# llm-d/llm-d-workload-variant-autoscaler

Measured on AMD Instinct MI355X. Metric: desired-replica accuracy + SLO-attainment %, Llama-3-8B synthetic QPS ramp, higher is better.
Workload: dtype bf16; 1 GPU; model=meta-llama/Llama-3.1-8B, global_batch=256, seq_len=150, parallelism=dp1, device=AMD Radeon Graphics

## Files before the change

### wva_amd/ops/csrc/attention.hip

```cpp
#include "common.h"

#include <type_traits>

#define HEAD_DIM 128
#define MAX_G 8
#define TILE 64
#define NUM_WAVES 4
#define ROW_DW 66
#define S_ROW 65

template <bool KV_FP8>
using kv_elem_t = std::conditional_t<KV_FP8, fp8_t, bf16>;

__device__ __forceinline__ long ws_row_offset(int b, int kvh, int g, int split,
                                              int num_kv_heads, int G,
                                              int num_splits) {
  return ((((long)b * num_kv_heads + kvh) * G + g) * num_splits + split) *
         (2 + HEAD_DIM);
}

__device__ __forceinline__ long pack8_fp8(const float* v, float inv_scale) {
  unsigned int lo = 0, hi = 0;
  lo = __builtin_amdgcn_cvt_pk_fp8_f32(v[0] * inv_scale, v[1] * inv_scale,
                                       lo, false);
// ... 35 lines not shown
#pragma unroll
      for (int i = 0; i < 8; ++i) {
        qf.bf[kk][i] = src[i];
        const bf16 bv = *reinterpret_cast<const bf16*>(&src[i]);
        qv[kk][i] = bf2f(bv);
      }
    }
  } else {
#pragma unroll
    for (int kk = 0; kk < 4; ++kk)
#pragma unroll
      for (int i = 0; i < 8; ++i) qf.bf[kk][i] = 0;
  }
  if constexpr (KV_FP8) {
    float amax = 0.0f;
#pragma unroll
    for (int kk = 0; kk < 4; ++kk)
#pragma unroll
      for (int i = 0; i < 8; ++i) amax = fmaxf(amax, fabsf(qv[kk][i]));
    amax = wave_reduce_max(amax);
    if (lane == 0) qmax_lds[wave] = amax;
    __syncthreads();
    float m0 = qmax_lds[0];
#pragma unroll
    for (int w2 = 1; w2 < NUM_WAVES; ++w2) m0 = fmaxf(m0, qmax_lds[w2]);
    qf.scale = fmaxf(m0 / 448.0f, 1e-12f);
    const float inv = 1.0f / qf.scale;
#pragma unroll
    for (int kk = 0; kk < 4; ++kk) qf.fp8[kk] = pack8_fp8(qv[kk], inv);
    __syncthreads();
  }
  return qf;
}

struct SoftmaxStep {
  float p;
  float corr;
};

__device__ __forceinline__ SoftmaxStep online_softmax_step(
    const float* __restrict__ s_row, int tn, int lane, float& m, float& s) {
  const bool live = lane < tn;
  const float score = live ? s_row[lane] : -INFINITY;
  const float tile_max = wave_reduce_max(score);
  const float m_new = fmaxf(m, tile_max);
  const float p = live ? __expf(score - m_new) : 0.0f;
  const float tile_sum = wave_reduce_sum(p);
  const float corr = (m == -INFINITY) ? 0.0f : __expf(m - m_new);
  s = s * corr + tile_sum;
  m = m_new;
  return {p, corr};
}

template <bool KV_FP8>
__global__ __launch_bounds__(256, 2) void gqa_decode_attn_v4_kernel(
    bf16* __restrict__ out,
    float* __restrict__ workspace,
    const bf16* __restrict__ q,
    const void* __restrict__ k_cache,
    const void* __restrict__ v_cache,
    const int* __restrict__ context_lens,
    const int num_q_heads,
    const int num_kv_heads,
    const int max_seq,
    const float scale) {
  const int b = blockIdx.x;
  const int kvh = blockIdx.y;
  const int split = blockIdx.z;
  const int num_splits = gridDim.z;
  const int G = num_q_heads / num_kv_heads;
  const int ctx = context_lens[b];

  const int lane = threadIdx.x & (WAVE_SIZE - 1);
  const int wave = threadIdx.x / WAVE_SIZE;
  const int frag_col = lane % 16;
  const int frag_k0 = 8 * (lane / 16);

  __shared__ float s_smem[MAX_G][S_ROW];
  __shared__ unsigned int v_smem[TILE * ROW_DW];
  __shared__ float p_smem[MAX_G][TILE];
  float* qmax_lds = nullptr;
  if constexpr (KV_FP8) {
    __shared__ float qmax_smem[NUM_WAVES];
    qmax_lds = qmax_smem;
  }

  const QFrags qf = load_q_frags<KV_FP8>(q, b, kvh, G, num_q_heads, lane,
                                         wave, frag_col, frag_k0, qmax_lds);

  const int heads_mine = (G > wave) ? (G - wave + NUM_WAVES - 1) / NUM_WAVES : 0;
  float m[2], s[2], acc[2][2];
#pragma unroll
  for (int j = 0; j < 2; ++j) {
    m[j] = -INFINITY;
    s[j] = 0.0f;
    acc[j][0] = acc[j][1] = 0.0f;
  }

  const long slab_off = ((long)b * num_kv_heads + kvh) * max_seq * HEAD_DIM;
  const auto* k_slab =
      reinterpret_cast<const kv_elem_t<KV_FP8>*>(k_cache) + slab_off;
  const auto* v_slab =
      reinterpret_cast<const kv_elem_t<KV_FP8>*>(v_cache) + slab_off;

  for (int t0 = split * TILE; t0 < ctx; t0 += num_splits * TILE) {
    const int tn = min(TILE, ctx - t0);

    if constexpr (KV_FP8) {
      const int tile_g8 = tn * (HEAD_DIM / 8);
      const fp8_t* v_src = v_slab + (long)t0 * HEAD_DIM;
      for (int idx = wave * WAVE_SIZE + lane; idx < tile_g8;
           idx += NUM_WAVES * WAVE_SIZE) {
        const int row = idx >> 4;
        const int d8 = (idx & 15) * 8;
        const unsigned short* src =
            reinterpret_cast<const unsigned short*>(
                v_src + (long)row * HEAD_DIM + d8);
        unsigned int* dst = &v_smem[row * ROW_DW + d8 / 2];
#pragma unroll
        for (int j = 0; j < 4; ++j) {
          const float2_vt f = unpk2_fp8(src[j]);
          const bf16x2 packed{f2bf(f[0]), f2bf(f[1])};
          dst[j] = *reinterpret_cast<const unsigned int*>(&packed);
        }
      }
    } else {
      typedef __attribute__((ext_vector_type(2))) unsigned int uint2_t;
      const int tile_u2 = tn * (HEAD_DIM / 4);
      const unsigned int* v_src =
          reinterpret_cast<const unsigned int*>(v_slab + (long)t0 * HEAD_DIM);
      for (int idx = wave * WAVE_SIZE + lane; idx < tile_u2;
           idx += NUM_WAVES * WAVE_SIZE) {
        const int row = idx >> 5;
        const int d2 = (idx & 31) * 2;
        const uint2_t val = *reinterpret_cast<const uint2_t*>(&v_src[idx * 2]);
        *reinterpret_cast<uint2_t*>(&v_smem[row * ROW_DW + d2]) = val;
      }
    }

    {
      const int prow = 16 * wave + (lane % 16);
      const int pos = t0 + prow;
      const int pos_c = pos < max_seq ? pos : max_seq - 1;
      const int k0 = frag_k0;
      f32x4_frag sf = {0.f, 0.f, 0.f, 0.f};
      if constexpr (KV_FP8) {
        const long* ksrc = reinterpret_cast<const long*>(
            k_slab + (long)pos_c * HEAD_DIM);
        const int l0 = k0 / 8;
#pragma unroll
        for (int kk = 0; kk < 4; ++kk) {
          const long a8 = ksrc[kk * 4 + l0];
          sf = __builtin_amdgcn_mfma_f32_16x16x32_fp8_fp8(
              a8, qf.fp8[kk], sf, 0, 0, 0);
        }
      } else {
#pragma unroll
        for (int kk = 0; kk < 4; ++kk) {
          bf16x8_frag a_frag;
          const short* src = reinterpret_cast<const short*>(
              k_slab + (long)pos_c * HEAD_DIM) + 32 * kk + k0;
#pragma unroll
          for (int i = 0; i < 8; ++i) a_frag[i] = src[i];
          sf = __builtin_amdgcn_mfma_f32_16x16x32_bf16(a_frag, qf.bf[kk],
                                                       sf, 0, 0, 0);
        }
      }
      const float s_eff = KV_FP8 ? scale * qf.scale : scale;
      const int g = lane & 15;
      if (g < G) {
#pragma unroll
        for (int i = 0; i < 4; ++i) {
          const int t = 16 * wave + (lane >> 4) * 4 + i;
          s_smem[g][t] = (t < tn) ? sf[i] * s_eff : -INFINITY;
        }
      }
    }
    __syncthreads();

    for (int j = 0; j < heads_mine; ++j) {
      const int g = wave + j * NUM_WAVES;
      const SoftmaxStep st = online_softmax_step(s_smem[g], tn, lane, m[j], s[j]);
      acc[j][0] *= st.corr;
      acc[j][1] *= st.corr;
      p_smem[g][lane] = st.p;
    }

    for (int j = 0; j < heads_mine; ++j) {
      const int g = wave + j * NUM_WAVES;
      const float* pg = p_smem[g];
      float a0 = acc[j][0], a1 = acc[j][1];
      for (int t = 0; t < tn; ++t) {
        const unsigned int vw = v_smem[t * ROW_DW + lane];
        const bf16x2 vv = *reinterpret_cast<const bf16x2*>(&vw);
        const float p = pg[t];
        a0 = fmaf(p, bf2f(vv.x), a0);
        a1 = fmaf(p, bf2f(vv.y), a1);
      }
      acc[j][0] = a0;
      acc[j][1] = a1;
    }
    __syncthreads();
  }

  if (num_splits == 1) {
    for (int j = 0; j < heads_mine; ++j) {
      const int g = wave + j * NUM_WAVES;
      const float inv = s[j] > 0.0f ? 1.0f / s[j] : 0.0f;
      bf16x2* orow = reinterpret_cast<bf16x2*>(
          out + ((long)b * num_q_heads + kvh * G + g) * HEAD_DIM);
      orow[lane] = bf16x2{f2bf(acc[j][0] * inv), f2bf(acc[j][1] * inv)};
    }
  } else {
    for (int j = 0; j < heads_mine; ++j) {
      const int g = wave + j * NUM_WAVES;
      float* wsp = workspace +
          ws_row_offset(b, kvh, g, split, num_kv_heads, G, num_splits);
      if (lane == 0) {
        wsp[0] = m[j];
        wsp[1] = s[j];
      }
      wsp[2 + 2 * lane] = acc[j][0];
      wsp[2 + 2 * lane + 1] = acc[j][1];
    }
  }
}

template <bool KV_FP8>
__global__ __launch_bounds__(256, 2) void gqa_decode_attn_v5_kernel(
    bf16* __restrict__ out,
    float* __restrict__ workspace,
    const bf16* __restrict__ q,
    const void* __restrict__ k_cache,
    const void* __restrict__ v_cache,
    const int* __restrict__ context_lens,
    const int num_q_heads,
    const int num_kv_heads,
    const int max_seq,
    const float scale) {
  const int b = blockIdx.x;
  const int kvh = blockIdx.y;
  const int split = blockIdx.z;
  const int num_splits = gridDim.z;
  const int G = num_q_heads / num_kv_heads;
  const int ctx = context_lens[b];

  const int lane = threadIdx.x & (WAVE_SIZE - 1);
  const int wave = threadIdx.x / WAVE_SIZE;
  const int frag_col = lane % 16;
  const int frag_k0 = 8 * (lane / 16);

  __shared__ float s_smem[MAX_G][S_ROW];
  __shared__ unsigned int v_smem[TILE * ROW_DW];
  __shared__ float p_smem[MAX_G][TILE];
  __shared__ float corr_smem[MAX_G];
  __shared__ float sum_smem[MAX_G];
  __shared__ float m_smem[MAX_G];
  float* qmax_lds = nullptr;
  if constexpr (KV_FP8) {
    __shared__ float qmax_smem[NUM_WAVES];
    qmax_lds = qmax_smem;
  }

  const QFrags qf = load_q_frags<KV_FP8>(q, b, kvh, G, num_q_heads, lane,
                                         wave, frag_col, frag_k0, qmax_lds);

  const int heads_mine = (G > wave) ? (G - wave + NUM_WAVES - 1) / NUM_WAVES : 0;
  float m[2], s[2];
#pragma unroll
  for (int j = 0; j < 2; ++j) {
    m[j] = -INFINITY;
    s[j] = 0.0f;
  }
  f32x4_frag acc_pv[2] = {f32x4_frag{0.f, 0.f, 0.f, 0.f},
                          f32x4_frag{0.f, 0.f, 0.f, 0.f}};

  const long slab_off = ((long)b * num_kv_heads + kvh) * max_seq * HEAD_DIM;
  const auto* k_slab =
      reinterpret_cast<const kv_elem_t<KV_FP8>*>(k_cache) + slab_off;
  const auto* v_slab =
      reinterpret_cast<const kv_elem_t<KV_FP8>*>(v_cache) + slab_off;

  for (int t0 = split * TILE; t0 < ctx; t0 += num_splits * TILE) {
    const int tn = min(TILE, ctx - t0);

    if constexpr (KV_FP8) {
      const int tile_g8 = tn * (HEAD_DIM / 8);
      const fp8_t* v_src = v_slab + (long)t0 * HEAD_DIM;
      for (int idx = wave * WAVE_SIZE + lane; idx < tile_g8;
           idx += NUM_WAVES * WAVE_SIZE) {
        const int row = idx >> 4;
        const int d8 = (idx & 15) * 8;
        const unsigned short* src =
            reinterpret_cast<const unsigned short*>(
                v_src + (long)row * HEAD_DIM + d8);
        unsigned int* dst = &v_smem[row * ROW_DW + d8 / 2];
#pragma unroll
        for (int j = 0; j < 4; ++j) {
          const float2_vt f = unpk2_fp8(src[j]);
          const bf16x2 packed{f2bf(f[0]), f2bf(f[1])};
          dst[j] = *reinterpret_cast<const unsigned int*>(&packed);
        }
      }
    } else {
      typedef __attribute__((ext_vector_type(2))) unsigned int uint2_t;
      const int tile_u2 = tn * (HEAD_DIM / 4);
      const unsigned int* v_src =
          reinterpret_cast<const unsigned int*>(v_slab + (long)t0 * HEAD_DIM);
      for (int idx = wave * WAVE_SIZE + lane; idx < tile_u2;
           idx += NUM_WAVES * WAVE_SIZE) {
        const int row = idx >> 5;
        const int d2 = (idx & 31) * 2;
        const uint2_t val = *reinterpret_cast<const uint2_t*>(&v_src[idx * 2]);
        *reinterpret_cast<uint2_t*>(&v_smem[row * ROW_DW + d2]) = val;
      }
    }

    {
      const int prow = 16 * wave + (lane % 16);
      const int pos = t0 + prow;
      const int pos_c = pos < max_seq ? pos : max_seq - 1;
      const int k0 = frag_k0;
      f32x4_frag sf = {0.f, 0.f, 0.f, 0.f};
      if constexpr (KV_FP8) {
        const long* ksrc = reinterpret_cast<const long*>(
            k_slab + (long)pos_c * HEAD_DIM);
        const int l0 = k0 / 8;
#pragma unroll
        for (int kk = 0; kk < 4; ++kk) {
          const long a8 = ksrc[kk * 4 + l0];
          sf = __builtin_amdgcn_mfma_f32_16x16x32_fp8_fp8(
              a8, qf.fp8[kk], sf, 0, 0, 0);
        }
      } else {
#pragma unroll
        for (int kk = 0; kk < 4; ++kk) {
          bf16x8_frag a_frag;
          const short* src = reinterpret_cast<const short*>(
              k_slab + (long)pos_c * HEAD_DIM) + 32 * kk + k0;
#pragma unroll
          for (int i = 0; i < 8; ++i) a_frag[i] = src[i];
          sf = __builtin_amdgcn_mfma_f32_16x16x32_bf16(a_frag, qf.bf[kk],
                                                       sf, 0, 0, 0);
        }
      }
      const float s_eff = KV_FP8 ? scale * qf.scale : scale;
      const int g = lane & 15;
      if (g < G) {
#pragma unroll
        for (int i = 0; i < 4; ++i) {
          const int t = 16 * wave + (lane >> 4) * 4 + i;
          s_smem[g][t] = (t < tn) ? sf[i] * s_eff : -INFINITY;
        }
      }
    }
    __syncthreads();

    for (int j = 0; j < heads_mine; ++j) {
      const int g = wave + j * NUM_WAVES;
      const SoftmaxStep st = online_softmax_step(s_smem[g], tn, lane, m[j], s[j]);
      p_smem[g][lane] = st.p;
      if (lane == 0) corr_smem[g] = st.corr;
    }
    __syncthreads();

    {
      bf16x8_frag p_frag[2];
#pragma unroll
      for (int kk = 0; kk < 2; ++kk) {
        const int g = lane % 16;
        const int pos0 = 32 * kk + 8 * (lane / 16);
        if (g < G) {
#pragma unroll
          for (int i = 0; i < 8; ++i)
            p_frag[kk][i] = f2bf_bits(p_smem[g][pos0 + i]);
        } else {
#pragma unroll
          for (int i = 0; i < 8; ++i) p_frag[kk][i] = 0;
        }
      }
      const unsigned short* v_u16 =
          reinterpret_cast<const unsigned short*>(v_smem);
#pragma unroll
      for (int nsub = 0; nsub < 2; ++nsub) {
        const int dim = 16 * (wave + 4 * nsub) + (lane % 16);
        f32x4_frag d = acc_pv[nsub];
#pragma unroll
        for (int i = 0; i < 4; ++i) {
          const int h = (lane >> 4) * 4 + i;
          d[i] *= (h < G) ? corr_smem[h] : 0.0f;
        }
#pragma unroll
        for (int kk = 0; kk < 2; ++kk) {
          bf16x8_frag v_frag;
          const int pos0 = 32 * kk + 8 * (lane / 16);
#pragma unroll
          for (int i = 0; i < 8; ++i) {
            const int t = pos0 + i;
            v_frag[i] = (t < tn)
                ? (short)v_u16[(t * ROW_DW + (dim >> 1)) * 2 + (dim & 1)]
                : (short)0;
          }
          d = __builtin_amdgcn_mfma_f32_16x16x32_bf16(p_frag[kk], v_frag, d,
                                                      0, 0, 0);
        }
        acc_pv[nsub] = d;
      }
    }
    __syncthreads();
  }

  for (int j = 0; j < heads_mine; ++j) {
    const int g = wave + j * NUM_WAVES;
    if (lane == 0) {
      sum_smem[g] = s[j];
      m_smem[g] = m[j];
    }
  }
  __syncthreads();

  if (num_splits == 1) {
#pragma unroll
    for (int nsub = 0; nsub < 2; ++nsub) {
      const int dim = 16 * (wave + 4 * nsub) + (lane & 15);
#pragma unroll
      for (int i = 0; i < 4; ++i) {
        const int h = (lane >> 4) * 4 + i;
        if (h >= G) continue;
        const float sv = sum_smem[h];
        const float inv = sv > 0.0f ? 1.0f / sv : 0.0f;
        out[((long)b * num_q_heads + kvh * G + h) * HEAD_DIM + dim] =
            f2bf(acc_pv[nsub][i] * inv);
      }
    }
  } else {
#pragma unroll
    for (int nsub = 0; nsub < 2; ++nsub) {
      const int dim = 16 * (wave + 4 * nsub) + (lane & 15);
#pragma unroll
      for (int i = 0; i < 4; ++i) {
        const int h = (lane >> 4) * 4 + i;
        if (h >= G) continue;
        float* wsp = workspace +
            ws_row_offset(b, kvh, h, split, num_kv_heads, G, num_splits);
        if (wave == 0 && nsub == 0 && (lane & 15) == 0) {
          wsp[0] = m_smem[h];
          wsp[1] = sum_smem[h];
        }
        wsp[2 + dim] = acc_pv[nsub][i];
      }
    }
  }
}

#define MERGE_WAVES 8
// ... 7 lines not shown
  const int h = blockIdx.y;
  const int G = num_q_heads / num_kv_heads;
  const int kvh = h / G;
  const int g = h % G;
  const int lane = threadIdx.x & 63;
  const int wave = threadIdx.x >> 6;

  __shared__ float sm_m[MERGE_WAVES];
  __shared__ float sm_s[MERGE_WAVES];
  __shared__ float sm_o[MERGE_WAVES][HEAD_DIM];

  const float* base = workspace +
      ws_row_offset(b, kvh, g, 0, num_kv_heads, G, num_splits);
  float M = -INFINITY;
  for (int sp = wave; sp < num_splits; sp += MERGE_WAVES) {
    M = fmaxf(M, base[sp * (2 + HEAD_DIM)]);
  }
  float S = 0.0f, o0 = 0.0f, o1 = 0.0f;
  for (int sp = wave; sp < num_splits; sp += MERGE_WAVES) {
    const float* wsp = base + sp * (2 + HEAD_DIM);
    const float mw = wsp[0];
    if (mw == -INFINITY) continue;
    const float f = __expf(mw - M);
    S += wsp[1] * f;
    o0 = fmaf(wsp[2 + 2 * lane], f, o0);
    o1 = fmaf(wsp[2 + 2 * lane + 1], f, o1);
  }
  if (lane == 0) {
    sm_m[wave] = M;
    sm_s[wave] = S;
  }
  sm_o[wave][2 * lane] = o0;
  sm_o[wave][2 * lane + 1] = o1;
  __syncthreads();

  if (wave != 0) return;
  float Mg = -INFINITY;
  for (int w = 0; w < MERGE_WAVES; ++w) Mg = fmaxf(Mg, sm_m[w]);
  float Sg = 0.0f;
  float g0 = 0.0f, g1 = 0.0f;
  for (int w = 0; w < MERGE_WAVES; ++w) {
    if (sm_m[w] == -INFINITY) continue;
    const float f = __expf(sm_m[w] - Mg);
    Sg += sm_s[w] * f;
    g0 = fmaf(sm_o[w][2 * lane], f, g0);
    g1 = fmaf(sm_o[w][2 * lane + 1], f, g1);
  }
  const float inv = Sg > 0.0f ? 1.0f / Sg : 0.0f;
  bf16x2* orow = reinterpret_cast<bf16x2*>(
      out + ((long)b * num_q_heads + h) * HEAD_DIM);
  orow[lane] = bf16x2{f2bf(g0 * inv), f2bf(g1 * inv)};
}

extern "C" int gqa_decode_attn_num_splits(int batch, int num_kv_heads,
                                          int max_ctx_hint) {
  const int base = batch * num_kv_heads;
  if (base >= 1792) return 1;
  int splits = 1792 / base;
  static int min_tiles = [] {
    const char* e = getenv("WVA_ATTN_MIN_TILES");
    int v = e ? atoi(e) : 8;
    return v > 0 ? v : 8;
  }();
  int cap = 16;
  if (max_ctx_hint > 0) {
    const int by_work = max_ctx_hint / (min_tiles * TILE);
    if (by_work > cap) cap = by_work;
  }
  if (splits > cap) splits = cap;
  const int max_useful = max_ctx_hint > 0 ? (max_ctx_hint + 2 * TILE - 1) / (2 * TILE) : splits;
  if (splits > max_useful && max_useful >= 1) splits = max_useful;
  return splits < 1 ? 1 : splits;
}

extern "C" void launch_gqa_decode_attn(
    void* out, void* workspace, const void* q, const void* k_cache,
    const void* v_cache, const int* context_lens, int batch, int num_q_heads,
    int num_kv_heads, int max_seq, int num_splits, float scale, int variant,
    int kv_fp8, hipStream_t stream) {
  const auto kernel =
      variant == 5 ? (kv_fp8 ? gqa_decode_attn_v5_kernel<true>
                             : gqa_decode_attn_v5_kernel<false>)
                   : (kv_fp8 ? gqa_decode_attn_v4_kernel<true>
                             : gqa_decode_attn_v4_kernel<false>);
  hipLaunchKernelGGL(kernel, dim3(batch, num_kv_heads, num_splits), dim3(256),
                     0, stream, (bf16*)out, (float*)workspace, (const bf16*)q,
                     k_cache, v_cache, context_lens, num_q_heads, num_kv_heads,
                     max_seq, scale);
  if (num_splits > 1) {
    hipLaunchKernelGGL(gqa_decode_attn_merge_kernel,
                       dim3(batch, num_q_heads), dim3(64 * MERGE_WAVES), 0,
                       stream, (bf16*)out, (const float*)workspace,
                       num_q_heads, num_kv_heads, num_splits);
  }
}
```

### wva_amd/ops/csrc/ops.cpp

```cpp

#include <torch/extension.h>
#include <hip/hip_runtime.h>
#include <c10/hip/HIPStream.h>

#include <string>

extern "C" void launch_rmsnorm(void* out, void* residual_out,
                               const void* input, const void* residual,
                               const void* weight, float eps, int rows,
                               int hidden, hipStream_t stream);
extern "C" void launch_rope(void* q, void* k, const int* positions, int tokens,
                            int num_q_heads, int num_k_heads, int head_dim,
                            float theta, hipStream_t stream);
extern "C" void launch_silu_mul(void* out, const void* gate, const void* up,
                                long n, hipStream_t stream);
extern "C" void launch_silu_mul_fused(void* out, const void* gate_up,
                                      long rows, long inter,
                                      hipStream_t stream);
extern "C" void launch_rope_append_kv_fp8(const void* qkv, void* q_out,
                                          void* k_cache, void* v_cache,
                                          const int* positions, int batch,
                                          int num_q_heads, int num_kv_heads,
                                          int head_dim, int max_seq,
                                          float theta, hipStream_t stream);
extern "C" void launch_rope_append_kv(const void* qkv, void* q_out,
                                      void* k_cache, void* v_cache,
                                      const int* positions, int batch,
                                      int num_q_heads, int num_kv_heads,
                                      int head_dim, int max_seq, float theta,
                                      hipStream_t stream);
extern "C" int gqa_decode_attn_num_splits(int batch, int num_kv_heads,
                                          int max_ctx_hint);
extern "C" int skinny_gemm_num_splits(int N, int K, int nt);
extern "C" void launch_prefill_attn_ex(void* out, const void* q,
                                       const void* k_cache,
                                       const void* v_cache, int batch,
                                       int seq, int num_q_heads,
                                       int num_kv_heads, int max_seq,
                                       float scale, int kv_fp8,
                                       hipStream_t stream);
extern "C" int skinny_gemm_tile_n(int M);
extern "C" void launch_skinny_gemm(void* c, void* ws, const void* a,
                                   const void* w, int M, int N, int K,
                                   int num_splits, hipStream_t stream);
extern "C" void launch_skinny_gemm_ex(void* c, void* ws, const void* a,
                                      const void* w, const float* w_scale,
                                      int M, int N, int K, int num_splits,
                                      int w_fp8, hipStream_t stream);
extern "C" void launch_gqa_decode_attn(void* out, void* workspace,
                                       const void* q, const void* k_cache,
                                       const void* v_cache,
                                       const int* context_lens, int batch,
                                       int num_q_heads, int num_kv_heads,
                                       int max_seq, int num_splits,
                                       float scale, int variant, int kv_fp8,
                                       hipStream_t stream);

extern "C" int moe_num_m_tiles(int TK, int E);
extern "C" int moe_down_num_splits(int TK, int E, int H, int I);
extern "C" void launch_moe_route(int* topk_idx, float* topk_w,
                                 int* expert_offsets, int* sorted_slots,
                                 const float* logits, int T, int E, int K,
                                 hipStream_t stream);
extern "C" void launch_moe_gate_up_swiglu(void* act, const void* x,
                                          const void* w,
                                          const int* expert_offsets,
                                          const int* sorted_slots, int T,
                                          int E, int top_k, int H, int I,
                                          hipStream_t stream);
extern "C" void launch_moe_down_combine(void* out, float* ws,
                                        const void* act, const void* w,
                                        const float* topk_w,
                                        const int* expert_offsets,
                                        const int* sorted_slots, int T,
                                        int E, int top_k, int H, int I,
                                        int num_splits, hipStream_t stream);

namespace {

hipStream_t current_stream() {
  return c10::hip::getCurrentHIPStream().stream();
}

void check_bf16_contig(const torch::Tensor& t, const char* name) {
  TORCH_CHECK(t.is_cuda(), name, " must be on GPU");
// ... 87 lines not shown
         (int)num_q_heads, (int)num_kv_heads, head_dim, max_seq,
         (float)theta, current_stream());
  return q_out;
}

torch::Tensor silu_mul_fused(torch::Tensor gate_up) {
  check_bf16_contig(gate_up, "gate_up");
  TORCH_CHECK(gate_up.dim() == 2 && gate_up.size(1) % 4 == 0,
              "gate_up must be [rows, 2*inter], inter even");
  const long rows = gate_up.size(0);
  const long inter = gate_up.size(1) / 2;
  auto out = torch::empty({rows, inter}, gate_up.options());
  launch_silu_mul_fused(out.data_ptr(), gate_up.data_ptr(), rows, inter,
                        current_stream());
  return out;
}

enum class AttnVariant { Auto, V4, V5 };

AttnVariant parse_attn_variant(const std::string& name) {
  TORCH_CHECK(name == "auto" || name == "v4" || name == "v5",
              "variant must be \"auto\", \"v4\" or \"v5\", got \"", name, "\"");
  return name == "v4"   ? AttnVariant::V4
         : name == "v5" ? AttnVariant::V5
                        : AttnVariant::Auto;
}

torch::Tensor gqa_decode_attn(torch::Tensor q, torch::Tensor k_cache,
                              torch::Tensor v_cache,
                              torch::Tensor context_lens, double scale,
                              const std::string& variant_name) {
  AttnVariant variant = parse_attn_variant(variant_name);
  check_bf16_contig(q, "q");
  const bool kv_fp8 = check_cache_contig(k_cache, "k_cache");
  TORCH_CHECK(check_cache_contig(v_cache, "v_cache") == kv_fp8,
              "k/v cache dtype mismatch");
  TORCH_CHECK(context_lens.is_cuda() &&
                  context_lens.scalar_type() == torch::kInt32,
              "context_lens must be int32 on GPU");
  TORCH_CHECK(q.dim() == 3, "q must be [B, Hq, D]");
  TORCH_CHECK(k_cache.dim() == 4,
              "k_cache must be [B, Hk, S, D] (head-major)");
  const int batch = q.size(0);
  const int num_q_heads = q.size(1);
  const int head_dim = q.size(2);
  const int num_kv_heads = k_cache.size(1);
  const int max_seq = k_cache.size(2);
  TORCH_CHECK(head_dim == 128, "head_dim must be 128 (Llama-3 family)");
  TORCH_CHECK(num_q_heads % num_kv_heads == 0, "Hq must divide by Hk");
  const int G = num_q_heads / num_kv_heads;
  TORCH_CHECK(G <= 8, "GQA group size must be <= 8");
  TORCH_CHECK(v_cache.sizes() == k_cache.sizes(), "k/v cache mismatch");
  auto out = torch::empty_like(q);
  const int num_splits =
      gqa_decode_attn_num_splits(batch, num_kv_heads, max_seq);
  if (variant == AttnVariant::Auto) {
    variant = (G >= 8 || num_splits == 1) ? AttnVariant::V5 : AttnVariant::V4;
  }
  torch::Tensor workspace;
  void* ws_ptr = nullptr;
  if (num_splits > 1) {
    workspace = torch::empty(
        {(long)batch * num_kv_heads * G * num_splits * (2 + head_dim)},
        q.options().dtype(torch::kFloat32));
    ws_ptr = workspace.data_ptr();
  }
  launch_gqa_decode_attn(out.data_ptr(), ws_ptr, q.data_ptr(),
                         k_cache.data_ptr(), v_cache.data_ptr(),
                         context_lens.data_ptr<int>(), batch, num_q_heads,
                         num_kv_heads, max_seq, num_splits, (float)scale,
                         variant == AttnVariant::V5 ? 5 : 4, kv_fp8 ? 1 : 0,
                         current_stream());
  return out;
}

torch::Tensor skinny_linear(torch::Tensor x, torch::Tensor w) {
  check_bf16_contig(x, "x");
  check_bf16_contig(w, "w");
  TORCH_CHECK(x.dim() == 2 && w.dim() == 2, "x [M,K], w [N,K]");
  const int M = x.size(0);
  const int K = x.size(1);
  const int N = w.size(0);
  TORCH_CHECK(w.size(1) == K, "K mismatch");
  TORCH_CHECK(M <= 64, "skinny_linear requires M <= 64");
  TORCH_CHECK(K % 128 == 0, "K must be a multiple of 128");
  auto y = torch::empty({M, N}, x.options());
  const int nt = skinny_gemm_tile_n(M);
  const int sk = skinny_gemm_num_splits(N, K, nt);
  torch::Tensor ws;
  void* ws_ptr = nullptr;
  if (sk > 1) {
    ws = torch::empty({(long)sk * M * N},
                      x.options().dtype(torch::kFloat32));
    ws_ptr = ws.data_ptr();
  }
  launch_skinny_gemm(y.data_ptr(), ws_ptr, x.data_ptr(), w.data_ptr(), M, N,
                     K, sk, current_stream());
  return y;
}

torch::Tensor skinny_linear_fp8(torch::Tensor x, torch::Tensor w,
                                torch::Tensor w_scale) {
  check_bf16_contig(x, "x");
  TORCH_CHECK(w.is_cuda() && w.is_contiguous() &&
                  w.scalar_type() == at::kFloat8_e4m3fn,
              "w must be contiguous float8_e4m3fn");
  TORCH_CHECK(w_scale.is_cuda() && w_scale.scalar_type() == torch::kFloat &&
                  w_scale.numel() == w.size(0),
              "w_scale must be float32 [N]");
  TORCH_CHECK(x.dim() == 2 && w.dim() == 2, "x [M,K], w [N,K]");
// ... 212 lines not shown
```

### wva_amd/ops/csrc/rope.hip

```cpp

#include "common.h"

__device__ __forceinline__ void rotate_pair(
    const bf16* src, bf16* dst, int d, int half, int head_dim, float pos,
    float theta) {
  const float inv_freq = __powf(theta, -2.0f * (float)d / (float)head_dim);
  const float angle = pos * inv_freq;
  float c, s;
  __sincosf(angle, &s, &c);
  const float x1 = bf2f(src[d]);
  const float x2 = bf2f(src[d + half]);
  dst[d] = f2bf(x1 * c - x2 * s);
  dst[d + half] = f2bf(x2 * c + x1 * s);
}

__global__ void rope_kernel(
    bf16* __restrict__ q,
    bf16* __restrict__ k,
    const int* __restrict__ positions,
    const int num_q_heads,
    const int num_k_heads,
    const int head_dim,
    const float theta) {
  const int token = blockIdx.x;
  const float pos = (float)positions[token];
  const int half = head_dim / 2;
  const int total = (num_q_heads + num_k_heads) * half;

  for (int idx = threadIdx.x; idx < total; idx += blockDim.x) {
    const int head = idx / half;
    const int d = idx % half;
    const bool is_q = head < num_q_heads;
    bf16* base = is_q
        ? q + (long)token * num_q_heads * head_dim + (long)head * head_dim
        : k + (long)token * num_k_heads * head_dim +
              (long)(head - num_q_heads) * head_dim;
    rotate_pair(base, base, d, half, head_dim, pos, theta);
  }
}

__global__ void rope_append_kv_kernel(
    const bf16* __restrict__ qkv,
    bf16* __restrict__ q_out,
    bf16* __restrict__ k_cache,
    bf16* __restrict__ v_cache,
    const int* __restrict__ positions,
    const int num_q_heads,
    const int num_kv_heads,
    const int head_dim,
    const int max_seq,
    const float theta) {
  const int b = blockIdx.x;
  const int pos_i = positions[b];
  const float pos = (float)pos_i;
  const int half = head_dim / 2;
  const long qkv_row = (long)b * (num_q_heads + 2 * num_kv_heads) * head_dim;

  const int rot_total = (num_q_heads + num_kv_heads) * half;
  for (int idx = threadIdx.x; idx < rot_total; idx += blockDim.x) {
    const int head = idx / half;
    const int d = idx % half;
    if (head < num_q_heads) {
      const bf16* src = qkv + qkv_row + (long)head * head_dim;
      bf16* dst = q_out + ((long)b * num_q_heads + head) * head_dim;
      rotate_pair(src, dst, d, half, head_dim, pos, theta);
    } else {
      const int kh = head - num_q_heads;
      const bf16* src = qkv + qkv_row + ((long)num_q_heads + kh) * head_dim;
      bf16* dst = k_cache +
          (((long)b * num_kv_heads + kh) * max_seq + pos_i) * head_dim;
      rotate_pair(src, dst, d, half, head_dim, pos, theta);
    }
  }
  const int v_total = num_kv_heads * half;
  const bf16x2* vsrc = reinterpret_cast<const bf16x2*>(
      qkv + qkv_row + (long)(num_q_heads + num_kv_heads) * head_dim);
  for (int idx = threadIdx.x; idx < v_total; idx += blockDim.x) {
    const int kh = idx / half;
    const int d2 = idx % half;
    bf16x2* dst = reinterpret_cast<bf16x2*>(
        v_cache + (((long)b * num_kv_heads + kh) * max_seq + pos_i) * head_dim);
    dst[d2] = vsrc[(long)kh * half + d2];
  }
}

__global__ void rope_append_kv_fp8_kernel(
    const bf16* __restrict__ qkv,
    bf16* __restrict__ q_out,
    fp8_t* __restrict__ k_cache,
    fp8_t* __restrict__ v_cache,
    const int* __restrict__ positions,
    const int num_q_heads,
    const int num_kv_heads,
    const int head_dim,
    const int max_seq,
    const float theta) {
  const int b = blockIdx.x;
  const int pos_i = positions[b];
  const float pos = (float)pos_i;
  const int half = head_dim / 2;
  const long qkv_row = (long)b * (num_q_heads + 2 * num_kv_heads) * head_dim;

  const int rot_total = (num_q_heads + num_kv_heads) * half;
  for (int idx = threadIdx.x; idx < rot_total; idx += blockDim.x) {
    const int head = idx / half;
    const int d = idx % half;
    if (head < num_q_heads) {
      const bf16* src = qkv + qkv_row + (long)head * head_dim;
      bf16* dst = q_out + ((long)b * num_q_heads + head) * head_dim;
      rotate_pair(src, dst, d, half, head_dim, pos, theta);
    } else {
      const int kh = head - num_q_heads;
      const bf16* src = qkv + qkv_row + ((long)num_q_heads + kh) * head_dim;
      const float inv_freq =
          __powf(theta, -2.0f * (float)d / (float)head_dim);
      const float angle = pos * inv_freq;
      float c, s;
      __sincosf(angle, &s, &c);
      const float x1 = bf2f(src[d]);
      const float x2 = bf2f(src[d + half]);
      fp8_t* dst = k_cache +
          (((long)b * num_kv_heads + kh) * max_seq + pos_i) * head_dim;
      dst[d] = f2fp8(x1 * c - x2 * s);
      dst[d + half] = f2fp8(x2 * c + x1 * s);
    }
  }
  const int v_total = num_kv_heads * half;
  const bf16x2* vsrc = reinterpret_cast<const bf16x2*>(
      qkv + qkv_row + (long)(num_q_heads + num_kv_heads) * head_dim);
  for (int idx = threadIdx.x; idx < v_total; idx += blockDim.x) {
    const int kh = idx / half;
    const int d2 = idx % half;
    const bf16x2 v2 = vsrc[(long)kh * half + d2];
    unsigned short* dst = reinterpret_cast<unsigned short*>(
        v_cache + (((long)b * num_kv_heads + kh) * max_seq + pos_i) * head_dim);
    dst[d2] = pk2_fp8(bf2f(v2.x), bf2f(v2.y));
  }
}

extern "C" void launch_rope_append_kv_fp8(
    const void* qkv, void* q_out, void* k_cache, void* v_cache,
    const int* positions, int batch, int num_q_heads, int num_kv_heads,
    int head_dim, int max_seq, float theta, hipStream_t stream) {
  dim3 grid(batch);
  dim3 block(256);
  hipLaunchKernelGGL(rope_append_kv_fp8_kernel, grid, block, 0, stream,
                     (const bf16*)qkv, (bf16*)q_out, (fp8_t*)k_cache,
                     (fp8_t*)v_cache, positions, num_q_heads, num_kv_heads,
                     head_dim, max_seq, theta);
}

extern "C" void launch_rope(
    void* q, void* k, const int* positions, int tokens, int num_q_heads,
    int num_k_heads, int head_dim, float theta, hipStream_t stream) {
  dim3 grid(tokens);
  dim3 block(256);
  hipLaunchKernelGGL(rope_kernel, grid, block, 0, stream, (bf16*)q, (bf16*)k,
                     positions, num_q_heads, num_k_heads, head_dim, theta);
}

extern "C" void launch_rope_append_kv(
    const void* qkv, void* q_out, void* k_cache, void* v_cache,
    const int* positions, int batch, int num_q_heads, int num_kv_heads,
    int head_dim, int max_seq, float theta, hipStream_t stream) {
  dim3 grid(batch);
  dim3 block(256);
  hipLaunchKernelGGL(rope_append_kv_kernel, grid, block, 0, stream,
                     (const bf16*)qkv, (bf16*)q_out, (bf16*)k_cache,
                     (bf16*)v_cache, positions, num_q_heads, num_kv_heads,
                     head_dim, max_seq, theta);
}
```

Baseline: 91.98 %.

## Prefetch KV tiles into registers, use LDS transpose reads, occupancy-based splits, per-head rope

Decode attention now issues the K and V global loads for the next tile into registers right after the score barrier, so memory latency overlaps with the softmax and PV work. V5 reads V fragments with ds_read_tr16 transpose loads instead of scalar gathers. Split count now comes from a runtime occupancy query rather than a hardcoded 1792 workgroups, and the v4 kernel gets a waves-per-EU hint. The rope/append kernel is rewritten to one wave per head on a 2D grid and merged into a single template. The register prefetch raises VGPR pressure, which could lower occupancy.

```diff
diff --git a/wva_amd/ops/csrc/attention.hip b/wva_amd/ops/csrc/attention.hip
--- a/wva_amd/ops/csrc/attention.hip
+++ b/wva_amd/ops/csrc/attention.hip
@@ -111,8 +111,79 @@
   return {p, corr};
 }
 
+typedef __attribute__((ext_vector_type(2))) unsigned int uint2_t;
+
 template <bool KV_FP8>
-__global__ __launch_bounds__(256, 2) void gqa_decode_attn_v4_kernel(
+struct KVTile {
+  static constexpr int ROW_BYTES = HEAD_DIM * (int)sizeof(kv_elem_t<KV_FP8>);
+  static constexpr int V_ROWS = NUM_WAVES * WAVE_SIZE * 8 / ROW_BYTES;
+  static constexpr int V_LOADS = TILE / V_ROWS;
+  static constexpr int V_THREADS_PER_ROW = ROW_BYTES / 8;
+  using k_frag_t = std::conditional_t<KV_FP8, long, bf16x8_frag>;
+  uint2_t v[V_LOADS];
+  k_frag_t k[4];
+};
+
+template <bool KV_FP8, bool WITH_V = true, bool WITH_K = true>
+__device__ __forceinline__ void issue_tile_loads(
+    KVTile<KV_FP8>& r, const kv_elem_t<KV_FP8>* __restrict__ k_slab,
+    const kv_elem_t<KV_FP8>* __restrict__ v_slab, int t0, int tn, int max_seq,
+    int tid, int k_row, int k0) {
+  using T = KVTile<KV_FP8>;
+  const int v_r0 = tid / T::V_THREADS_PER_ROW;
+  const char* v_col = reinterpret_cast<const char*>(v_slab) +
+                      (long)t0 * T::ROW_BYTES +
+                      (tid % T::V_THREADS_PER_ROW) * 8;
+  if constexpr (WITH_V) {
+#pragma unroll
+    for (int i = 0; i < T::V_LOADS; ++i) {
+      const int row = min(v_r0 + T::V_ROWS * i, tn - 1);
+      r.v[i] = *reinterpret_cast<const uint2_t*>(v_col + row * T::ROW_BYTES);
+    }
+  }
+  const int pos = t0 + k_row;
+  const int pos_c = pos < max_seq ? pos : max_seq - 1;
+  const char* k_src = reinterpret_cast<const char*>(k_slab) +
+                      (long)pos_c * T::ROW_BYTES +
+                      k0 * (int)sizeof(kv_elem_t<KV_FP8>);
+  if constexpr (WITH_K) {
+#pragma unroll
+    for (int kk = 0; kk < 4; ++kk)
+      r.k[kk] = *reinterpret_cast<const typename T::k_frag_t*>(
+          k_src + 32 * kk * (int)sizeof(kv_elem_t<KV_FP8>));
+  }
+}
+
+template <bool KV_FP8>
+__device__ __forceinline__ void stage_v_tile(unsigned int* v_smem,
+                                             const KVTile<KV_FP8>& r, int tn,
+                                             int tid) {
+  using T = KVTile<KV_FP8>;
+  const int v_r0 = tid / T::V_THREADS_PER_ROW;
+  const int dw = (tid % T::V_THREADS_PER_ROW) * (KV_FP8 ? 4 : 2);
+  unsigned int* dst0 = &v_smem[v_r0 * ROW_DW + dw];
+#pragma unroll
+  for (int i = 0; i < T::V_LOADS; ++i) {
+    const bool live = v_r0 + T::V_ROWS * i < tn;
+    unsigned int* dst = dst0 + T::V_ROWS * i * ROW_DW;
+    if constexpr (KV_FP8) {
+#pragma unroll
+      for (int j = 0; j < 4; ++j) {
+        const unsigned int w = live ? r.v[i][j >> 1] : 0u;
+        const float2_vt f =
+            unpk2_fp8((unsigned short)((j & 1) ? (w >> 16) : (w & 0xffffu)));
+        const bf16x2 packed{f2bf(f[0]), f2bf(f[1])};
+        dst[j] = *reinterpret_cast<const unsigned int*>(&packed);
+      }
+    } else {
+      *reinterpret_cast<uint2_t*>(dst) = live ? r.v[i] : uint2_t{0u, 0u};
+    }
+  }
+}
+
+template <bool KV_FP8>
+__global__ __launch_bounds__(256) __attribute__((amdgpu_waves_per_eu(5)))
+void gqa_decode_attn_v4_kernel(
     bf16* __restrict__ out,
     float* __restrict__ workspace,
     const bf16* __restrict__ q,
@@ -162,66 +233,32 @@
   const auto* v_slab =
       reinterpret_cast<const kv_elem_t<KV_FP8>*>(v_cache) + slab_off;
 
+  const int k_row = 16 * wave + frag_col;
+  constexpr bool AHEAD_V = KV_FP8;
+  KVTile<KV_FP8> kv;
+  if (split * TILE < ctx)
+    issue_tile_loads<KV_FP8, AHEAD_V, true>(kv, k_slab, v_slab, split * TILE,
+                             min(TILE, ctx - split * TILE), max_seq,
+                             threadIdx.x, k_row, frag_k0);
+
   for (int t0 = split * TILE; t0 < ctx; t0 += num_splits * TILE) {
     const int tn = min(TILE, ctx - t0);
 
-    if constexpr (KV_FP8) {
-      const int tile_g8 = tn * (HEAD_DIM / 8);
-      const fp8_t* v_src = v_slab + (long)t0 * HEAD_DIM;
-      for (int idx = wave * WAVE_SIZE + lane; idx < tile_g8;
-           idx += NUM_WAVES * WAVE_SIZE) {
-        const int row = idx >> 4;
-        const int d8 = (idx & 15) * 8;
-        const unsigned short* src =
-            reinterpret_cast<const unsigned short*>(
-                v_src + (long)row * HEAD_DIM + d8);
-        unsigned int* dst = &v_smem[row * ROW_DW + d8 / 2];
-#pragma unroll
-        for (int j = 0; j < 4; ++j) {
-          const float2_vt f = unpk2_fp8(src[j]);
-          const bf16x2 packed{f2bf(f[0]), f2bf(f[1])};
-          dst[j] = *reinterpret_cast<const unsigned int*>(&packed);
-        }
-      }
-    } else {
-      typedef __attribute__((ext_vector_type(2))) unsigned int uint2_t;
-      const int tile_u2 = tn * (HEAD_DIM / 4);
-      const unsigned int* v_src =
-          reinterpret_cast<const unsigned int*>(v_slab + (long)t0 * HEAD_DIM);
-      for (int idx = wave * WAVE_SIZE + lane; idx < tile_u2;
-           idx += NUM_WAVES * WAVE_SIZE) {
-        const int row = idx >> 5;
-        const int d2 = (idx & 31) * 2;
-        const uint2_t val = *reinterpret_cast<const uint2_t*>(&v_src[idx * 2]);
-        *reinterpret_cast<uint2_t*>(&v_smem[row * ROW_DW + d2]) = val;
-      }
-    }
+    if constexpr (!AHEAD_V)
+      issue_tile_loads<KV_FP8, true, false>(kv, k_slab, v_slab, t0, tn,
+                                            max_seq, threadIdx.x, k_row,
+                                            frag_k0);
+    stage_v_tile<KV_FP8>(v_smem, kv, tn, threadIdx.x);
 
     {
-      const int prow = 16 * wave + (lane % 16);
-      const int pos = t0 + prow;
-      const int pos_c = pos < max_seq ? pos : max_seq - 1;
-      const int k0 = frag_k0;
       f32x4_frag sf = {0.f, 0.f, 0.f, 0.f};
-      if constexpr (KV_FP8) {
-        const long* ksrc = reinterpret_cast<const long*>(
-            k_slab + (long)pos_c * HEAD_DIM);
-        const int l0 = k0 / 8;
-#pragma unroll
-        for (int kk = 0; kk < 4; ++kk) {
-          const long a8 = ksrc[kk * 4 + l0];
+#pragma unroll
+      for (int kk = 0; kk < 4; ++kk) {
+        if constexpr (KV_FP8) {
           sf = __builtin_amdgcn_mfma_f32_16x16x32_fp8_fp8(
-              a8, qf.fp8[kk], sf, 0, 0, 0);
-        }
-      } else {
-#pragma unroll
-        for (int kk = 0; kk < 4; ++kk) {
-          bf16x8_frag a_frag;
-          const short* src = reinterpret_cast<const short*>(
-              k_slab + (long)pos_c * HEAD_DIM) + 32 * kk + k0;
-#pragma unroll
-          for (int i = 0; i < 8; ++i) a_frag[i] = src[i];
-          sf = __builtin_amdgcn_mfma_f32_16x16x32_bf16(a_frag, qf.bf[kk],
+              kv.k[kk], qf.fp8[kk], sf, 0, 0, 0);
+        } else {
+          sf = __builtin_amdgcn_mfma_f32_16x16x32_bf16(kv.k[kk], qf.bf[kk],
                                                        sf, 0, 0, 0);
         }
       }
@@ -236,6 +273,11 @@
       }
     }
     __syncthreads();
+    if (t0 + num_splits * TILE < ctx) {
+      const int t1 = t0 + num_splits * TILE;
+      issue_tile_loads<KV_FP8, AHEAD_V, true>(kv, k_slab, v_slab, t1, min(TILE, ctx - t1),
+                               max_seq, threadIdx.x, k_row, frag_k0);
+    }
 
     for (int j = 0; j < heads_mine; ++j) {
       const int g = wave + j * NUM_WAVES;
@@ -310,7 +352,7 @@
   const int frag_k0 = 8 * (lane / 16);
 
   __shared__ float s_smem[MAX_G][S_ROW];
-  __shared__ unsigned int v_smem[TILE * ROW_DW];
+  __shared__ __attribute__((aligned(16))) unsigned int v_smem[TILE * ROW_DW];
   __shared__ float p_smem[MAX_G][TILE];
   __shared__ float corr_smem[MAX_G];
   __shared__ float sum_smem[MAX_G];
@@ -340,66 +382,27 @@
   const auto* v_slab =
       reinterpret_cast<const kv_elem_t<KV_FP8>*>(v_cache) + slab_off;
 
+  const int k_row = 16 * wave + frag_col;
+  KVTile<KV_FP8> kv;
+  if (split * TILE < ctx)
+    issue_tile_loads<KV_FP8>(kv, k_slab, v_slab, split * TILE,
+                             min(TILE, ctx - split * TILE), max_seq,
+                             threadIdx.x, k_row, frag_k0);
+
   for (int t0 = split * TILE; t0 < ctx; t0 += num_splits * TILE) {
     const int tn = min(TILE, ctx - t0);
 
-    if constexpr (KV_FP8) {
-      const int tile_g8 = tn * (HEAD_DIM / 8);
-      const fp8_t* v_src = v_slab + (long)t0 * HEAD_DIM;
-      for (int idx = wave * WAVE_SIZE + lane; idx < tile_g8;
-           idx += NUM_WAVES * WAVE_SIZE) {
-        const int row = idx >> 4;
-        const int d8 = (idx & 15) * 8;
-        const unsigned short* src =
-            reinterpret_cast<const unsigned short*>(
-                v_src + (long)row * HEAD_DIM + d8);
-        unsigned int* dst = &v_smem[row * ROW_DW + d8 / 2];
-#pragma unroll
-        for (int j = 0; j < 4; ++j) {
-          const float2_vt f = unpk2_fp8(src[j]);
-          const bf16x2 packed{f2bf(f[0]), f2bf(f[1])};
-          dst[j] = *reinterpret_cast<const unsigned int*>(&packed);
-        }
-      }
-    } else {
-      typedef __attribute__((ext_vector_type(2))) unsigned int uint2_t;
-      const int tile_u2 = tn * (HEAD_DIM / 4);
-      const unsigned int* v_src =
-          reinterpret_cast<const unsigned int*>(v_slab + (long)t0 * HEAD_DIM);
-      for (int idx = wave * WAVE_SIZE + lane; idx < tile_u2;
-           idx += NUM_WAVES * WAVE_SIZE) {
-        const int row = idx >> 5;
-        const int d2 = (idx & 31) * 2;
-        const uint2_t val = *reinterpret_cast<const uint2_t*>(&v_src[idx * 2]);
-        *reinterpret_cast<uint2_t*>(&v_smem[row * ROW_DW + d2]) = val;
-      }
-    }
+    stage_v_tile<KV_FP8>(v_smem, kv, tn, threadIdx.x);
 
     {
-      const int prow = 16 * wave + (lane % 16);
-      const int pos = t0 + prow;
-      const int pos_c = pos < max_seq ? pos : max_seq - 1;
-      const int k0 = frag_k0;
       f32x4_frag sf = {0.f, 0.f, 0.f, 0.f};
-      if constexpr (KV_FP8) {
-        const long* ksrc = reinterpret_cast<const long*>(
-            k_slab + (long)pos_c * HEAD_DIM);
-        const int l0 = k0 / 8;
-#pragma unroll
-        for (int kk = 0; kk < 4; ++kk) {
-          const long a8 = ksrc[kk * 4 + l0];
+#pragma unroll
+      for (int kk = 0; kk < 4; ++kk) {
+        if constexpr (KV_FP8) {
           sf = __builtin_amdgcn_mfma_f32_16x16x32_fp8_fp8(
-              a8, qf.fp8[kk], sf, 0, 0, 0);
-        }
-      } else {
-#pragma unroll
-        for (int kk = 0; kk < 4; ++kk) {
-          bf16x8_frag a_frag;
-          const short* src = reinterpret_cast<const short*>(
-              k_slab + (long)pos_c * HEAD_DIM) + 32 * kk + k0;
-#pragma unroll
-          for (int i = 0; i < 8; ++i) a_frag[i] = src[i];
-          sf = __builtin_amdgcn_mfma_f32_16x16x32_bf16(a_frag, qf.bf[kk],
+              kv.k[kk], qf.fp8[kk], sf, 0, 0, 0);
+        } else {
+          sf = __builtin_amdgcn_mfma_f32_16x16x32_bf16(kv.k[kk], qf.bf[kk],
                                                        sf, 0, 0, 0);
         }
       }
@@ -414,6 +417,11 @@
       }
     }
     __syncthreads();
+    if (t0 + num_splits * TILE < ctx) {
+      const int t1 = t0 + num_splits * TILE;
+      issue_tile_loads<KV_FP8>(kv, k_slab, v_slab, t1, min(TILE, ctx - t1),
+                               max_seq, threadIdx.x, k_row, frag_k0);
+    }
 
     for (int j = 0; j < heads_mine; ++j) {
       const int g = wave + j * NUM_WAVES;
@@ -438,11 +446,15 @@
           for (int i = 0; i < 8; ++i) p_frag[kk][i] = 0;
         }
       }
+      typedef __attribute__((ext_vector_type(4))) short short4_t;
+      typedef __attribute__((address_space(3))) short4_t lds_short4_t;
       const unsigned short* v_u16 =
           reinterpret_cast<const unsigned short*>(v_smem);
+      const unsigned short* v_tr =
+          v_u16 + (8 * (lane / 16) + ((lane & 15) >> 2)) * (ROW_DW * 2) +
+          4 * (lane & 3);
 #pragma unroll
       for (int nsub = 0; nsub < 2; ++nsub) {
-        const int dim = 16 * (wave + 4 * nsub) + (lane % 16);
         f32x4_frag d = acc_pv[nsub];
 #pragma unroll
         for (int i = 0; i < 4; ++i) {
@@ -451,15 +463,14 @@
         }
 #pragma unroll
         for (int kk = 0; kk < 2; ++kk) {
-          bf16x8_frag v_frag;
-          const int pos0 = 32 * kk + 8 * (lane / 16);
-#pragma unroll
-          for (int i = 0; i < 8; ++i) {
-            const int t = pos0 + i;
-            v_frag[i] = (t < tn)
-                ? (short)v_u16[(t * ROW_DW + (dim >> 1)) * 2 + (dim & 1)]
-                : (short)0;
-          }
+          const unsigned short* blk =
+              v_tr + 32 * kk * (ROW_DW * 2) + 16 * (wave + 4 * nsub);
+          const short4_t lo = __builtin_amdgcn_ds_read_tr16_b64_v4i16(
+              (lds_short4_t*)blk);
+          const short4_t hi = __builtin_amdgcn_ds_read_tr16_b64_v4i16(
+              (lds_short4_t*)(blk + 4 * (ROW_DW * 2)));
+          const bf16x8_frag v_frag = {lo[0], lo[1], lo[2], lo[3],
+                                      hi[0], hi[1], hi[2], hi[3]};
           d = __builtin_amdgcn_mfma_f32_16x16x32_bf16(p_frag[kk], v_frag, d,
                                                       0, 0, 0);
         }
@@ -573,11 +584,48 @@
   orow[lane] = bf16x2{f2bf(g0 * inv), f2bf(g1 * inv)};
 }
 
+using attn_kernel_t = void (*)(bf16*, float*, const bf16*, const void*,
+                               const void*, const int*, int, int, int, float);
+
+static attn_kernel_t attn_kernel(int variant, int kv_fp8) {
+  return variant == 5 ? (kv_fp8 ? gqa_decode_attn_v5_kernel<true>
+                                : gqa_decode_attn_v5_kernel<false>)
+                      : (kv_fp8 ? gqa_decode_attn_v4_kernel<true>
+                                : gqa_decode_attn_v4_kernel<false>);
+}
+
+static int attn_resident_workgroups(int variant, int kv_fp8) {
+  struct Table {
+    int wgs[2][2];
+    Table() {
+      int dev = 0, cus = 0;
+      const bool ok =
+          hipGetDevice(&dev) == hipSuccess &&
+          hipDeviceGetAttribute(&cus, hipDeviceAttributeMultiprocessorCount,
+                                dev) == hipSuccess;
+      for (int v5 = 0; v5 < 2; ++v5)
+        for (int f8 = 0; f8 < 2; ++f8) {
+          int per_cu = 0;
+          if (!ok || hipOccupancyMaxActiveBlocksPerMultiprocessor(
+                         &per_cu, attn_kernel(v5 ? 5 : 4, f8),
+                         NUM_WAVES * WAVE_SIZE, 0) != hipSuccess)
+            per_cu = 0;
+          wgs[v5][f8] = per_cu * cus;
+        }
+    }
+  };
+  static const Table table;
+  return table.wgs[variant == 5][kv_fp8 != 0];
+}
+
 extern "C" int gqa_decode_attn_num_splits(int batch, int num_kv_heads,
-                                          int max_ctx_hint) {
+                                          int max_ctx_hint, int variant,
+                                          int kv_fp8) {
+  const int target = attn_resident_workgroups(variant, kv_fp8);
+  if (target <= 0) return 0;
   const int base = batch * num_kv_heads;
-  if (base >= 1792) return 1;
-  int splits = 1792 / base;
+  if (base >= target) return 1;
+  int splits = target / base;
   static int min_tiles = [] {
     const char* e = getenv("WVA_ATTN_MIN_TILES");
     int v = e ? atoi(e) : 8;
@@ -599,11 +647,7 @@
     const void* v_cache, const int* context_lens, int batch, int num_q_heads,
     int num_kv_heads, int max_seq, int num_splits, float scale, int variant,
     int kv_fp8, hipStream_t stream) {
-  const auto kernel =
-      variant == 5 ? (kv_fp8 ? gqa_decode_attn_v5_kernel<true>
-                             : gqa_decode_attn_v5_kernel<false>)
-                   : (kv_fp8 ? gqa_decode_attn_v4_kernel<true>
-                             : gqa_decode_attn_v4_kernel<false>);
+  const attn_kernel_t kernel = attn_kernel(variant, kv_fp8);
   hipLaunchKernelGGL(kernel, dim3(batch, num_kv_heads, num_splits), dim3(256),
                      0, stream, (bf16*)out, (float*)workspace, (const bf16*)q,
                      k_cache, v_cache, context_lens, num_q_heads, num_kv_heads,
diff --git a/wva_amd/ops/csrc/ops.cpp b/wva_amd/ops/csrc/ops.cpp
--- a/wva_amd/ops/csrc/ops.cpp
+++ b/wva_amd/ops/csrc/ops.cpp
@@ -30,7 +30,8 @@
                                       int head_dim, int max_seq, float theta,
                                       hipStream_t stream);
 extern "C" int gqa_decode_attn_num_splits(int batch, int num_kv_heads,
-                                          int max_ctx_hint);
+                                          int max_ctx_hint, int variant,
+                                          int kv_fp8);
 extern "C" int skinny_gemm_num_splits(int N, int K, int nt);
 extern "C" void launch_prefill_attn_ex(void* out, const void* q,
                                        const void* k_cache,
@@ -224,10 +225,20 @@
   TORCH_CHECK(G <= 8, "GQA group size must be <= 8");
   TORCH_CHECK(v_cache.sizes() == k_cache.sizes(), "k/v cache mismatch");
   auto out = torch::empty_like(q);
-  const int num_splits =
-      gqa_decode_attn_num_splits(batch, num_kv_heads, max_seq);
+  const auto splits_of = [&](AttnVariant v) {
+    const int n = gqa_decode_attn_num_splits(batch, num_kv_heads, max_seq,
+                                             v == AttnVariant::V5 ? 5 : 4,
+                                             kv_fp8 ? 1 : 0);
+    TORCH_CHECK(n >= 1, "decode attention: occupancy query failed");
+    return n;
+  };
+  int num_splits;
   if (variant == AttnVariant::Auto) {
-    variant = (G >= 8 || num_splits == 1) ? AttnVariant::V5 : AttnVariant::V4;
+    variant = G >= 8 ? AttnVariant::V5 : AttnVariant::V4;
+    num_splits = splits_of(variant);
+    if (num_splits == 1) variant = AttnVariant::V5;
+  } else {
+    num_splits = splits_of(variant);
   }
   torch::Tensor workspace;
   void* ws_ptr = nullptr;
diff --git a/wva_amd/ops/csrc/rope.hip b/wva_amd/ops/csrc/rope.hip
--- a/wva_amd/ops/csrc/rope.hip
+++ b/wva_amd/ops/csrc/rope.hip
@@ -39,11 +39,13 @@
   }
 }
 
-__global__ void rope_append_kv_kernel(
+#define ROPE_WAVES 4
+template <bool KV_FP8>
+__global__ __launch_bounds__(ROPE_WAVES * WAVE_SIZE) void rope_append_kv_kernel(
     const bf16* __restrict__ qkv,
     bf16* __restrict__ q_out,
-    bf16* __restrict__ k_cache,
-    bf16* __restrict__ v_cache,
+    void* __restrict__ k_cache,
+    void* __restrict__ v_cache,
     const int* __restrict__ positions,
     const int num_q_heads,
     const int num_kv_heads,
@@ -51,103 +53,80 @@
     const int max_seq,
     const float theta) {
   const int b = blockIdx.x;
+  const int lane = threadIdx.x & (WAVE_SIZE - 1);
+  const int head = blockIdx.y * ROPE_WAVES + threadIdx.x / WAVE_SIZE;
+  const int heads = num_q_heads + 2 * num_kv_heads;
+  if (head >= heads) return;
   const int pos_i = positions[b];
   const float pos = (float)pos_i;
   const int half = head_dim / 2;
-  const long qkv_row = (long)b * (num_q_heads + 2 * num_kv_heads) * head_dim;
+  const bf16* src = qkv + ((long)b * heads + head) * head_dim;
 
-  const int rot_total = (num_q_heads + num_kv_heads) * half;
-  for (int idx = threadIdx.x; idx < rot_total; idx += blockDim.x) {
-    const int head = idx / half;
-    const int d = idx % half;
-    if (head < num_q_heads) {
-      const bf16* src = qkv + qkv_row + (long)head * head_dim;
-      bf16* dst = q_out + ((long)b * num_q_heads + head) * head_dim;
+  if (head < num_q_heads) {
+    bf16* dst = q_out + ((long)b * num_q_heads + head) * head_dim;
+    for (int d = lane; d < half; d += WAVE_SIZE)
       rotate_pair(src, dst, d, half, head_dim, pos, theta);
+    return;
+  }
+  const bool is_k = head < num_q_heads + num_kv_heads;
+  const int kh = head - num_q_heads - (is_k ? 0 : num_kv_heads);
+  const long row = (((long)b * num_kv_heads + kh) * max_seq + pos_i) * head_dim;
+  if (is_k) {
+    if constexpr (KV_FP8) {
+      fp8_t* dst = reinterpret_cast<fp8_t*>(k_cache) + row;
+      for (int d = lane; d < half; d += WAVE_SIZE) {
+        const float inv_freq =
+            __powf(theta, -2.0f * (float)d / (float)head_dim);
+        const float angle = pos * inv_freq;
+        float c, s;
+        __sincosf(angle, &s, &c);
+        const float x1 = bf2f(src[d]);
+        const float x2 = bf2f(src[d + half]);
+        dst[d] = f2fp8(x1 * c - x2 * s);
+        dst[d + half] = f2fp8(x2 * c + x1 * s);
+      }
     } else {
-      const int kh = head - num_q_heads;
-      const bf16* src = qkv + qkv_row + ((long)num_q_heads + kh) * head_dim;
-      bf16* dst = k_cache +
-          (((long)b * num_kv_heads + kh) * max_seq + pos_i) * head_dim;
-      rotate_pair(src, dst, d, half, head_dim, pos, theta);
+      bf16* dst = reinterpret_cast<bf16*>(k_cache) + row;
+      for (int d = lane; d < half; d += WAVE_SIZE)
+        rotate_pair(src, dst, d, half, head_dim, pos, theta);
     }
-  }
-  const int v_total = num_kv_heads * half;
-  const bf16x2* vsrc = reinterpret_cast<const bf16x2*>(
-      qkv + qkv_row + (long)(num_q_heads + num_kv_heads) * head_dim);
-  for (int idx = threadIdx.x; idx < v_total; idx += blockDim.x) {
-    const int kh = idx / half;
-    const int d2 = idx % half;
-    bf16x2* dst = reinterpret_cast<bf16x2*>(
-        v_cache + (((long)b * num_kv_heads + kh) * max_seq + pos_i) * head_dim);
-    dst[d2] = vsrc[(long)kh * half + d2];
+  } else {
+    const bf16x2* vsrc = reinterpret_cast<const bf16x2*>(src);
+    for (int d2 = lane; d2 < half; d2 += WAVE_SIZE) {
+      if constexpr (KV_FP8) {
+        const bf16x2 v2 = vsrc[d2];
+        reinterpret_cast<unsigned short*>(
+            reinterpret_cast<fp8_t*>(v_cache) + row)[d2] =
+            pk2_fp8(bf2f(v2.x), bf2f(v2.y));
+      } else {
+        reinterpret_cast<bf16x2*>(reinterpret_cast<bf16*>(v_cache) + row)[d2] =
+            vsrc[d2];
+      }
+    }
   }
 }
 
-__global__ void rope_append_kv_fp8_kernel(
-    const bf16* __restrict__ qkv,
-    bf16* __restrict__ q_out,
-    fp8_t* __restrict__ k_cache,
-    fp8_t* __restrict__ v_cache,
-    const int* __restrict__ positions,
-    const int num_q_heads,
-    const int num_kv_heads,
-    const int head_dim,
-    const int max_seq,
-    const float theta) {
-  const int b = blockIdx.x;
-  const int pos_i = positions[b];
-  const float pos = (float)pos_i;
-  const int half = head_dim / 2;
-  const long qkv_row = (long)b * (num_q_heads + 2 * num_kv_heads) * head_dim;
-
-  const int rot_total = (num_q_heads + num_kv_heads) * half;
-  for (int idx = threadIdx.x; idx < rot_total; idx += blockDim.x) {
-    const int head = idx / half;
-    const int d = idx % half;
-    if (head < num_q_heads) {
-      const bf16* src = qkv + qkv_row + (long)head * head_dim;
-      bf16* dst = q_out + ((long)b * num_q_heads + head) * head_dim;
-      rotate_pair(src, dst, d, half, head_dim, pos, theta);
-    } else {
-      const int kh = head - num_q_heads;
-      const bf16* src = qkv + qkv_row + ((long)num_q_heads + kh) * head_dim;
-      const float inv_freq =
-          __powf(theta, -2.0f * (float)d / (float)head_dim);
-      const float angle = pos * inv_freq;
-      float c, s;
-      __sincosf(angle, &s, &c);
-      const float x1 = bf2f(src[d]);
-      const float x2 = bf2f(src[d + half]);
-      fp8_t* dst = k_cache +
-          (((long)b * num_kv_heads + kh) * max_seq + pos_i) * head_dim;
-      dst[d] = f2fp8(x1 * c - x2 * s);
-      dst[d + half] = f2fp8(x2 * c + x1 * s);
-    }
-  }
-  const int v_total = num_kv_heads * half;
-  const bf16x2* vsrc = reinterpret_cast<const bf16x2*>(
-      qkv + qkv_row + (long)(num_q_heads + num_kv_heads) * head_dim);
-  for (int idx = threadIdx.x; idx < v_total; idx += blockDim.x) {
-    const int kh = idx / half;
-    const int d2 = idx % half;
-    const bf16x2 v2 = vsrc[(long)kh * half + d2];
-    unsigned short* dst = reinterpret_cast<unsigned short*>(
-        v_cache + (((long)b * num_kv_heads + kh) * max_seq + pos_i) * head_dim);
-    dst[d2] = pk2_fp8(bf2f(v2.x), bf2f(v2.y));
-  }
+template <bool KV_FP8>
+static void launch_rope_append_kv_impl(
+    const void* qkv, void* q_out, void* k_cache, void* v_cache,
+    const int* positions, int batch, int num_q_heads, int num_kv_heads,
+    int head_dim, int max_seq, float theta, hipStream_t stream) {
+  const int heads = num_q_heads + 2 * num_kv_heads;
+  dim3 grid(batch, (heads + ROPE_WAVES - 1) / ROPE_WAVES);
+  dim3 block(ROPE_WAVES * WAVE_SIZE);
+  hipLaunchKernelGGL(rope_append_kv_kernel<KV_FP8>, grid, block, 0, stream,
+                     (const bf16*)qkv, (bf16*)q_out, k_cache, v_cache,
+                     positions, num_q_heads, num_kv_heads, head_dim, max_seq,
+                     theta);
 }
 
 extern "C" void launch_rope_append_kv_fp8(
     const void* qkv, void* q_out, void* k_cache, void* v_cache,
     const int* positions, int batch, int num_q_heads, int num_kv_heads,
     int head_dim, int max_seq, float theta, hipStream_t stream) {
-  dim3 grid(batch);
-  dim3 block(256);
-  hipLaunchKernelGGL(rope_append_kv_fp8_kernel, grid, block, 0, stream,
-                     (const bf16*)qkv, (bf16*)q_out, (fp8_t*)k_cache,
-                     (fp8_t*)v_cache, positions, num_q_heads, num_kv_heads,
-                     head_dim, max_seq, theta);
+  launch_rope_append_kv_impl<true>(qkv, q_out, k_cache, v_cache, positions,
+                                   batch, num_q_heads, num_kv_heads, head_dim,
+                                   max_seq, theta, stream);
 }
 
 extern "C" void launch_rope(
@@ -163,10 +142,7 @@
     const void* qkv, void* q_out, void* k_cache, void* v_cache,
     const int* positions, int batch, int num_q_heads, int num_kv_heads,
     int head_dim, int max_seq, float theta, hipStream_t stream) {
-  dim3 grid(batch);
-  dim3 block(256);
-  hipLaunchKernelGGL(rope_append_kv_kernel, grid, block, 0, stream,
-                     (const bf16*)qkv, (bf16*)q_out, (bf16*)k_cache,
-                     (bf16*)v_cache, positions, num_q_heads, num_kv_heads,
-                     head_dim, max_seq, theta);
+  launch_rope_append_kv_impl<false>(qkv, q_out, k_cache, v_cache, positions,
+                                    batch, num_q_heads, num_kv_heads, head_dim,
+                                    max_seq, theta, stream);
 }
```

Measured after the change: 75.22 %. 0.818x the previous value.
